# Fil/nd4js

Measured on AMD Instinct MI355X. Metric: fp64 GFLOP/s: matmul N=4096 & SVD N=2048; % of MFMA/HBM peak, higher is better.
Workload: dtype f64; 1 GPU; matmul 4096x4096x4096 fp64, one matrix pair per GPU (BASELINE configs[1]); parallelism=batch-sharded x1, no collective, inputs=uniform(-1,1) seeds 5/6, HBM-resident

## Files before the change

nd4js_amd/csrc/gemm.hip:

```cpp
#include "nd4hip_internal.h"
#include <cstdlib>

typedef double d4 __attribute__((ext_vector_type(4)));
typedef double d2 __attribute__((ext_vector_type(2)));

namespace {

constexpr int BM = 128, BN = 128, BK = 16;
constexpr int LDR = BK + 1;
constexpr int LDK = BN + 16;
constexpr int TILE = BK * LDK;
constexpr int NXCD = 8, GROUP_M = 8;

struct GemmArgs {
  const double* A; const double* B; double* C;
  int M, N, K;
  long lda, ldb, ldc, sA, sB, sC;
  double alpha, beta;
  int tiles_m, tiles_n;
  int lower;
  int kchunk;
  double* Cpart;
};

template <bool VEC, bool FULL>
__device__ __forceinline__ void load_row(d2 (&r)[4], const double* __restrict__ P, long ld,
                                         int x0, int X, int k0, int K, int t) {
  const int kc = k0 + ((t & 7) << 1);
#pragma unroll
  for (int q = 0; q < 4; q++) {
    const int x = x0 + q * 32 + (t >> 3);
    const double* p = P + (long)x * ld + kc;
    if (FULL) {
      r[q] = *reinterpret_cast<const d2*>(p);
    } else if (VEC) {
      d2 v = {0.0, 0.0};
      if (x < X && kc < K) v = *reinterpret_cast<const d2*>(p);
      r[q] = v;
    } else {
      double a = 0.0, b = 0.0;
      if (x < X && kc < K) a = p[0];
      if (x < X && kc + 1 < K) b = p[1];
      r[q].x = a; r[q].y = b;
    }
  }
}
__device__ __forceinline__ void store_row(double* S, const d2 (&r)[4], int t) {
  const int kc = (t & 7) << 1;
#pragma unroll
  for (int q = 0; q < 4; q++) {
    double* s = S + (q * 32 + (t >> 3)) * LDR + kc;
    s[0] = r[q].x; s[1] = r[q].y;
  }
}
template <bool VEC, bool FULL>
__device__ __forceinline__ void load_kmaj(d2 (&r)[4], const double* __restrict__ P, long ld,
                                          int x0, int X, int k0, int K, int t) {
  const int k = k0 + (t >> 4);
#pragma unroll
  for (int q = 0; q < 4; q++) {
    const int x = x0 + q * 32 + ((t & 15) << 1);
    const double* p = P + (long)k * ld + x;
    if (FULL) {
      r[q] = *reinterpret_cast<const d2*>(p);
    } else if (VEC) {
      d2 v = {0.0, 0.0};
      if (k < K && x < X) v = *reinterpret_cast<const d2*>(p);
      r[q] = v;
    } else {
      double a = 0.0, b = 0.0;
      if (k < K && x < X) a = p[0];
      if (k < K && x + 1 < X) b = p[1];
      r[q].x = a; r[q].y = b;
    }
  }
}
__device__ __forceinline__ void store_kmaj(double* S, const d2 (&r)[4], int t) {
#pragma unroll
  for (int q = 0; q < 4; q++)
    *reinterpret_cast<d2*>(S + (t >> 4) * LDK + q * 32 + ((t & 15) << 1)) = r[q];
}

template <bool FULL, bool BETA>
__device__ __forceinline__ void store_c(const d4 (&acc)[4][4], double* __restrict__ c0, long ldc, int rows, int cols, double alpha, double beta) {
#pragma unroll
  for (int i = 0; i < 4; i++)
#pragma unroll
    for (int j = 0; j < 4; j++)
#pragma unroll
      for (int r = 0; r < 4; r++)
        if (FULL || (i * 16 + 4 * r < rows && j * 16 < cols)) {
          double* c = c0 + (long)(i * 16 + 4 * r) * ldc + j * 16;
          double v = alpha * acc[i][j][r];
          if (BETA) v += beta * *c;
          *c = v;
        }
}

template <bool TA, bool TB, bool VEC, bool FULL>
__global__ __launch_bounds__(256, 2) void dgemm_kernel(GemmArgs g) {
  __shared__ __attribute__((aligned(16))) double lds[4 * TILE];

  const int nwg = g.tiles_m * g.tiles_n;
  int wg;
  {
    const int bid = blockIdx.x, xcd = bid % NXCD, within = bid / NXCD;
    const int q = nwg / NXCD, r = nwg % NXCD;
    wg = (xcd < r ? xcd * (q + 1) : r * (q + 1) + (xcd - r) * q) + within;
  }
  const int per_group = GROUP_M * g.tiles_n;
  const int first_m = (wg / per_group) * GROUP_M;
  const int gsz = min(g.tiles_m - first_m, GROUP_M);
  const int tm = first_m + (wg % per_group) % gsz;
  const int tn = (wg % per_group) / gsz;
  const int m0 = tm * BM, n0 = tn * BN;
  if (g.lower && n0 > m0 + BM - 1) return;

  const long bz = blockIdx.y;
  const double* __restrict__ A = g.A + bz * g.sA;
  const double* __restrict__ B = g.B + bz * g.sB;
  double* __restrict__ C = g.C + bz * g.sC;
  int kbeg = 0, kend = g.K;
  long ldc = g.ldc;
  double alpha = g.alpha, beta = g.beta;
  if (g.kchunk > 0) {
    kbeg = blockIdx.z * g.kchunk; kend = min(g.K, kbeg + g.kchunk);
    C = g.Cpart + ((long)blockIdx.z * gridDim.y + bz) * g.M * g.N;
    ldc = g.N; alpha = 1.0; beta = 0.0;
  }

  const int t = threadIdx.x, lane = t & 63, wave = t >> 6;
  const int wm = (wave >> 1) * 64, wn = (wave & 1) * 64;
  const int fx = lane & 15, fk = lane >> 4;

  d4 acc[4][4];
#pragma unroll
  for (int i = 0; i < 4; i++)
#pragma unroll
    for (int j = 0; j < 4; j++) acc[i][j] = d4{0.0, 0.0, 0.0, 0.0};

  d2 ra[4], rb[4];
  auto gload = [&](int k0) {
    if (TA) load_kmaj<VEC, FULL>(ra, A, g.lda, m0, g.M, k0, kend, t); else load_row<VEC, FULL>(ra, A, g.lda, m0, g.M, k0, kend, t);
    if (TB) load_row<VEC, FULL>(rb, B, g.ldb, n0, g.N, k0, kend, t);  else load_kmaj<VEC, FULL>(rb, B, g.ldb, n0, g.N, k0, kend, t);
  };
  auto sstore = [&](int buf) {
    double* sa = lds + buf * 2 * TILE; double* sb = sa + TILE;
    if (TA) store_kmaj(sa, ra, t); else store_row(sa, ra, t);
    if (TB) store_row(sb, rb, t);  else store_kmaj(sb, rb, t);
  };

  const double* fa = lds + (TA ? fk * LDK + wm + fx : (wm + fx) * LDR + fk);
  const double* fb = lds + TILE + (TB ? (wn + fx) * LDR + fk : fk * LDK + wn + fx);
  auto fread = [&](double (&a)[4], double (&b)[4], int buf, int kk) __attribute__((always_inline)) {
#pragma unroll
    for (int i = 0; i < 4; i++) a[i] = fa[buf * 2 * TILE + (TA ? kk * 4 * LDK + i * 16 : i * 16 * LDR + kk * 4)];
#pragma unroll
    for (int j = 0; j < 4; j++) b[j] = fb[buf * 2 * TILE + (TB ? j * 16 * LDR + kk * 4 : kk * 4 * LDK + j * 16)];
    __builtin_amdgcn_sched_barrier(0);
  };
  auto mma = [&](const double (&a)[4], const double (&b)[4]) __attribute__((always_inline)) {
#pragma unroll
    for (int i = 0; i < 4; i++)
#pragma unroll
      for (int j = 0; j < 4; j++)
        acc[i][j] = __builtin_amdgcn_mfma_f64_16x16x4f64(a[i], b[j], acc[i][j], 0, 0, 0);
    __builtin_amdgcn_sched_barrier(0);
  };

  const int nk = (kend - kbeg + BK - 1) / BK;
  gload(kbeg);
  sstore(0);
  if (nk > 1) gload(kbeg + BK);
  __syncthreads();

  double a0[4], b0[4], a1[4], b1[4];
  fread(a0, b0, 0, 0);
  auto kstep = [&](int cur, int kt, bool more, bool more2) __attribute__((always_inline)) {
    fread(a1, b1, cur, 1); mma(a0, b0);
    fread(a0, b0, cur, 2); mma(a1, b1);
    fread(a1, b1, cur, 3);
    if (more) { sstore(cur ^ 1); __builtin_amdgcn_sched_barrier(0); }
    mma(a0, b0);
    if (more) {
      __syncthreads();
      if (more2) gload(kbeg + (kt + 2) * BK);
      fread(a0, b0, cur ^ 1, 0);
    }
    mma(a1, b1);
  };
  int kt = 0;
  for (; kt + 2 < nk; kt += 2) {
    kstep(0, kt, true, true);
    kstep(1, kt + 1, true, kt + 3 < nk);
  }
  if (kt < nk) kstep(0, kt, kt + 1 < nk, false);
  if (kt + 1 < nk) kstep(1, kt + 1, false, false);

  double* c0 = C + (long)(m0 + wm + fk) * ldc + n0 + wn + fx;
  if (beta != 0.0) store_c<FULL, true>(acc, c0, ldc, g.M - (m0 + wm + fk), g.N - (n0 + wn + fx), alpha, beta);
  else             store_c<FULL, false>(acc, c0, ldc, g.M - (m0 + wm + fk), g.N - (n0 + wn + fx), alpha, beta);
}

constexpr int SK_RT = 1;
constexpr int SK_CT = 2;
constexpr int SK_BM = 4 * 16 * SK_RT, SK_BN = 16 * SK_CT, SK_KSTEPS = 8;

template <bool TB>
__global__ __launch_bounds__(256, 4) void dgemm_smallk_kernel(GemmArgs g) {
  const int tm = blockIdx.x / g.tiles_n, tn = blockIdx.x % g.tiles_n;
  const int m0 = tm * SK_BM, n0 = tn * SK_BN;
  if (g.lower && n0 > m0 + SK_BM - 1) return;
  const int lane = threadIdx.x & 63, w = threadIdx.x >> 6;
  const int fx = lane & 15, fk = lane >> 4;
  const int rbase = m0 + w * 16 * SK_RT;
  if (rbase >= g.M) return;
  const long bz = blockIdx.y;
  const double* __restrict__ A = g.A + bz * g.sA;
  const double* __restrict__ B = g.B + bz * g.sB;
  double* __restrict__ C = g.C + bz * g.sC;
  const int nk = (g.K + 3) >> 2;

  d4 acc[SK_RT][SK_CT];
  const double scale = (g.beta == 0.0) ? 0.0 : g.beta / g.alpha;
#pragma unroll
  for (int i = 0; i < SK_RT; i++)
#pragma unroll
    for (int j = 0; j < SK_CT; j++) {
      const int col = n0 + j * 16 + fx;
#pragma unroll
      for (int r = 0; r < 4; r++) {
        const int row = rbase + i * 16 + fk + 4 * r;
        double c = 0.0;
        if (scale != 0.0 && row < g.M && col < g.N) c = scale * C[(long)row * g.ldc + col];
        acc[i][j][r] = c;
      }
    }
  double a[SK_RT][SK_KSTEPS], b[SK_CT][SK_KSTEPS];
#pragma unroll
  for (int i = 0; i < SK_RT; i++) {
    const int row = rbase + i * 16 + fx;
    const double* ap = A + (long)row * g.lda + fk;
#pragma unroll
    for (int kk = 0; kk < SK_KSTEPS; kk++) a[i][kk] = (row < g.M && kk * 4 + fk < g.K) ? ap[kk * 4] : 0.0;
  }
#pragma unroll
  for (int j = 0; j < SK_CT; j++) {
    const int col = n0 + j * 16 + fx;
#pragma unroll
    for (int kk = 0; kk < SK_KSTEPS; kk++) {
      const int k = kk * 4 + fk;
      double v = 0.0;
      if (col < g.N && k < g.K) v = TB ? B[(long)col * g.ldb + k] : B[(long)k * g.ldb + col];
      b[j][kk] = v;
    }
  }
#pragma unroll
  for (int kk = 0; kk < SK_KSTEPS; kk++)
    if (kk < nk) {
#pragma unroll
      for (int i = 0; i < SK_RT; i++)
#pragma unroll
        for (int j = 0; j < SK_CT; j++) acc[i][j] = __builtin_amdgcn_mfma_f64_16x16x4f64(a[i][kk], b[j][kk], acc[i][j], 0, 0, 0);
    }
  const double alpha = g.alpha;
#pragma unroll
  for (int i = 0; i < SK_RT; i++)
#pragma unroll
    for (int j = 0; j < SK_CT; j++) {
      const int col = n0 + j * 16 + fx;
#pragma unroll
      for (int r = 0; r < 4; r++) {
        const int row = rbase + i * 16 + fk + 4 * r;
        if (row < g.M && col < g.N) C[(long)row * g.ldc + col] = alpha * acc[i][j][r];
      }
    }
}

bool smallk_ok(const GemmArgs& g, bool transA) {
  return !transA && g.K >= 1 && g.K <= 4 * SK_KSTEPS && (g.alpha == 1.0 || g.alpha == -1.0) &&
         (g.beta == 0.0 || g.beta == 1.0 || g.beta == -1.0);
}
template <bool TB>
int launch_smallk(nd4hip_handle* h, GemmArgs g, int64_t batch) {
  g.tiles_m = (g.M + SK_BM - 1) / SK_BM; g.tiles_n = (g.N + SK_BN - 1) / SK_BN;
  ND4_CHECK_ARG((int64_t)g.tiles_m * g.tiles_n < (1ll << 31), "nd4_gemm: too many tiles");
  hipLaunchKernelGGL((dgemm_smallk_kernel<TB>), dim3((unsigned)(g.tiles_m * g.tiles_n), (unsigned)batch, 1), dim3(256, 1, 1), 0, h->stream, g);
  ND4_HIP(hipGetLastError());
  return 0;
}

__global__ __launch_bounds__(256) void dgemm_splitk_reduce(const double* __restrict__ part, int nsplit, long per_split, int M, int N,
                                                            double alpha, double beta, double* __restrict__ Cm, long ldc, long sC) {
  const long b = blockIdx.y;
  const long e = blockIdx.x * 256l + threadIdx.x;
  if (e >= (long)M * N) return;
  double s = 0.0;
  for (int z = 0; z < nsplit; z++) s += part[z * per_split + b * (long)M * N + e];
  double* c = Cm + b * sC + (e / N) * ldc + e % N;
  double v = alpha * s;
  if (beta != 0.0) v += beta * *c;
  *c = v;
}


template <bool TA, bool TB>
int launch(nd4hip_handle* h, const GemmArgs& g, bool vec, int64_t batch) {
  const unsigned nsplit = g.kchunk > 0 ? (unsigned)((g.K + g.kchunk - 1) / g.kchunk) : 1u;
  dim3 grid((unsigned)(g.tiles_m * g.tiles_n), (unsigned)batch, nsplit), block(256, 1, 1);
  const bool full = vec && g.M % BM == 0 && g.N % BN == 0 && g.K % BK == 0 && g.K > 0;
  if (full)     hipLaunchKernelGGL((dgemm_kernel<TA, TB, true, true>), grid, block, 0, h->stream, g);
  else if (vec) hipLaunchKernelGGL((dgemm_kernel<TA, TB, true, false>), grid, block, 0, h->stream, g);
  else          hipLaunchKernelGGL((dgemm_kernel<TA, TB, false, false>), grid, block, 0, h->stream, g);
  ND4_HIP(hipGetLastError());
  return 0;
}

}

int nd4_gemm(nd4hip_handle* h, bool transA, bool transB, int64_t M, int64_t N, int64_t K,
             double alpha, const double* A, int64_t lda, int64_t sA,
             const double* B, int64_t ldb, int64_t sB,
             double beta, double* C, int64_t ldc, int64_t sC, int64_t batch) {
  if (M <= 0 || N <= 0 || batch <= 0) return 0;
  ND4_CHECK_ARG(K >= 0 && M < (1 << 30) && N < (1 << 30) && K < (1 << 30), "nd4_gemm: extent out of range");
  ND4_CHECK_ARG(batch <= 65535, "nd4_gemm: batch %lld exceeds 65535 per launch", (long long)batch);
  GemmArgs g;
  g.A = A; g.B = B; g.C = C; g.M = (int)M; g.N = (int)N; g.K = (int)K;
  g.lda = lda; g.ldb = ldb; g.ldc = ldc; g.sA = sA; g.sB = sB; g.sC = sC;
  g.alpha = alpha; g.beta = beta; g.lower = 0; g.kchunk = 0; g.Cpart = nullptr;
  g.tiles_m = (int)((M + BM - 1) / BM); g.tiles_n = (int)((N + BN - 1) / BN);
  ND4_CHECK_ARG((int64_t)g.tiles_m * g.tiles_n < (1ll << 31), "nd4_gemm: too many tiles");
  if (smallk_ok(g, transA)) return transB ? launch_smallk<true>(h, g, batch) : launch_smallk<false>(h, g, batch);
  Nd4WsScope scope(h);
  const int64_t tiles = (int64_t)g.tiles_m * g.tiles_n * batch;
  int nsplit = 1;
  if (tiles <= 160 && K >= 512) {
    int64_t want = 384 / tiles;
    if (want > K / 256) want = K / 256;
    if (want > 32) want = 32;
    if (want >= 2) {
      int64_t kc = ((K + want - 1) / want + BK - 1) / BK * BK;
      nsplit = (int)((K + kc - 1) / kc);
      void* p = nullptr;
      ND4_TRY(nd4_ws_alloc(h, sizeof(double) * (size_t)nsplit * (size_t)batch * (size_t)M * (size_t)N, &p));
      g.kchunk = (int)kc; g.Cpart = static_cast<double*>(p);
    }
  }
  auto even = [](int64_t v) { return (v & 1) == 0; };
  auto al16 = [](const void* p) { return (reinterpret_cast<uintptr_t>(p) & 15) == 0; };
  const bool vec = al16(A) && al16(B) && even(lda) && even(ldb) && even(sA) && even(sB) &&
                   even(transA ? M : K) && even(transB ? K : N);
  if (transA) ND4_TRY((transB ? launch<true, true>(h, g, vec, batch) : launch<true, false>(h, g, vec, batch)));
  else        ND4_TRY((transB ? launch<false, true>(h, g, vec, batch) : launch<false, false>(h, g, vec, batch)));
  if (g.kchunk > 0) {
    hipLaunchKernelGGL(dgemm_splitk_reduce, dim3((unsigned)((M * N + 255) / 256), (unsigned)batch), dim3(256), 0, h->stream,
                       g.Cpart, nsplit, (long)batch * M * N, (int)M, (int)N, alpha, beta, C, (long)ldc, (long)sC);
    ND4_HIP(hipGetLastError());
  }
  return 0;
}

int nd4_syrk_lower(nd4hip_handle* h, int64_t N, int64_t K, double alpha, const double* A, int64_t lda, int64_t sA,
                   double beta, double* C, int64_t ldc, int64_t sC, int64_t batch) {
  return nd4_gemm_nt_lower(h, N, K, alpha, A, lda, sA, A, lda, sA, beta, C, ldc, sC, batch);
}
int nd4_gemm_nt_lower(nd4hip_handle* h, int64_t N, int64_t K, double alpha, const double* A, int64_t lda, int64_t sA,
                      const double* B, int64_t ldb, int64_t sB, double beta, double* C, int64_t ldc, int64_t sC, int64_t batch) {
  if (N <= 0 || batch <= 0) return 0;
  ND4_CHECK_ARG(K >= 0 && N < (1 << 30) && K < (1 << 30), "nd4_gemm_nt_lower: extent out of range");
  ND4_CHECK_ARG(batch <= 65535, "nd4_gemm_nt_lower: batch %lld exceeds 65535 per launch", (long long)batch);
  GemmArgs g;
  g.A = A; g.B = B; g.C = C; g.M = (int)N; g.N = (int)N; g.K = (int)K;
  g.lda = lda; g.ldb = ldb; g.ldc = ldc; g.sA = sA; g.sB = sB; g.sC = sC;
  g.alpha = alpha; g.beta = beta; g.lower = 1; g.kchunk = 0; g.Cpart = nullptr;
  if (smallk_ok(g, false)) return launch_smallk<true>(h, g, batch);
  g.tiles_m = (int)((N + BM - 1) / BM); g.tiles_n = g.tiles_m;
  auto ok = [](const double* p, int64_t ld, int64_t st) { return (reinterpret_cast<uintptr_t>(p) & 15) == 0 && (ld & 1) == 0 && (st & 1) == 0; };
  const bool vec = ok(A, lda, sA) && ok(B, ldb, sB) && (K & 1) == 0;
  return launch<false, true>(h, g, vec, batch);
}
```

Baseline: 70950 GFLOP/s.

## Make DGEMM kernel persistent with grid-stride tile walk and prefetched next tile

Replaces the one-workgroup-per-tile launch with a persistent grid sized to resident occupancy times CU count. Each workgroup walks tiles, batches and split-K chunks with a grid stride, and loads the next tile's first K slice before storing the current C tile. The aim is to cut workgroup launch and tail overhead and to overlap the epilogue with the next tile's loads. It adds per-item index math read from the kernarg segment and optional timestamp instrumentation behind a compile flag. It may also disturb the XCD/group-M tile mapping locality for 4096 matrices.

New measurement: 67840 GFLOP/s. 4.4% lower.

```diff
diff --git a/nd4js_amd/csrc/gemm.hip b/nd4js_amd/csrc/gemm.hip
--- a/nd4js_amd/csrc/gemm.hip
+++ b/nd4js_amd/csrc/gemm.hip
@@ -21,7 +21,20 @@
   int lower;
   int kchunk;
   double* Cpart;
+  int batch, work;
+#ifdef ND4_GEMM_STAMPS
+  unsigned long long* stamps;
+#endif
 };
+
+#ifdef ND4_GEMM_STAMPS
+constexpr int STAMP_WORDS = 32;
+unsigned long long* g_stamps = nullptr;
+int g_stamps_one_trip = 0;
+#define ND4_STAMP(i) do { if (st && t == 0) { __builtin_amdgcn_sched_barrier(0); st[i] = wall_clock64(); __builtin_amdgcn_sched_barrier(0); } } while (0)
+#else
+#define ND4_STAMP(i) do { } while (0)
+#endif
 
 template <bool VEC, bool FULL>
 __device__ __forceinline__ void load_row(d2 (&r)[4], const double* __restrict__ P, long ld,
@@ -101,44 +114,47 @@
 __global__ __launch_bounds__(256, 2) void dgemm_kernel(GemmArgs g) {
   __shared__ __attribute__((aligned(16))) double lds[4 * TILE];
 
-  const int nwg = g.tiles_m * g.tiles_n;
-  int wg;
-  {
-    const int bid = blockIdx.x, xcd = bid % NXCD, within = bid / NXCD;
+  int m0, n0, kbeg, kend;
+  const double* A; const double* B; double* C;
+  const long ldc = g.kchunk > 0 ? g.N : g.ldc;
+  const double alpha = g.kchunk > 0 ? 1.0 : g.alpha, beta = g.kchunk > 0 ? 0.0 : g.beta;
+  typedef const __attribute__((address_space(4))) GemmArgs* KernArgs;
+  auto item = [&](int v) {
+    KernArgs ka = (KernArgs)__builtin_amdgcn_kernarg_segment_ptr();
+    asm volatile("" : "+s"(ka));
+    const int tiles_m = ka->tiles_m, tiles_n = ka->tiles_n, nwg = tiles_m * tiles_n, batch = ka->batch, kchunk = ka->kchunk;
+    const int bid = v % nwg, rest = v / nwg, xcd = bid % NXCD, within = bid / NXCD;
     const int q = nwg / NXCD, r = nwg % NXCD;
-    wg = (xcd < r ? xcd * (q + 1) : r * (q + 1) + (xcd - r) * q) + within;
-  }
-  const int per_group = GROUP_M * g.tiles_n;
-  const int first_m = (wg / per_group) * GROUP_M;
-  const int gsz = min(g.tiles_m - first_m, GROUP_M);
-  const int tm = first_m + (wg % per_group) % gsz;
-  const int tn = (wg % per_group) / gsz;
-  const int m0 = tm * BM, n0 = tn * BN;
-  if (g.lower && n0 > m0 + BM - 1) return;
-
-  const long bz = blockIdx.y;
-  const double* __restrict__ A = g.A + bz * g.sA;
-  const double* __restrict__ B = g.B + bz * g.sB;
-  double* __restrict__ C = g.C + bz * g.sC;
-  int kbeg = 0, kend = g.K;
-  long ldc = g.ldc;
-  double alpha = g.alpha, beta = g.beta;
-  if (g.kchunk > 0) {
-    kbeg = blockIdx.z * g.kchunk; kend = min(g.K, kbeg + g.kchunk);
-    C = g.Cpart + ((long)blockIdx.z * gridDim.y + bz) * g.M * g.N;
-    ldc = g.N; alpha = 1.0; beta = 0.0;
-  }
+    const int wg = (xcd < r ? xcd * (q + 1) : r * (q + 1) + (xcd - r) * q) + within;
+    const int per_group = GROUP_M * tiles_n;
+    const int first_m = (wg / per_group) * GROUP_M;
+    const int gsz = min(tiles_m - first_m, GROUP_M);
+    m0 = (first_m + (wg % per_group) % gsz) * BM;
+    n0 = ((wg % per_group) / gsz) * BN;
+    const long bz = rest % batch, z = rest / batch;
+    A = ka->A + bz * ka->sA; B = ka->B + bz * ka->sB; C = ka->C + bz * ka->sC;
+    kbeg = 0; kend = ka->K;
+    if (kchunk > 0) {
+      kbeg = (int)z * kchunk; kend = min(kend, kbeg + kchunk);
+      C = ka->Cpart + (z * batch + bz) * ka->M * ka->N;
+    }
+    return !(ka->lower && n0 > m0 + BM - 1);
+  };
+  auto next_item = [&](int v) {
+    KernArgs ka = (KernArgs)__builtin_amdgcn_kernarg_segment_ptr();
+    asm volatile("" : "+s"(ka));
+    for (const int work = ka->work; v < work; v += gridDim.x)
+      if (item(v)) return v;
+    return -1;
+  };
+  int v = next_item(blockIdx.x);
+  if (v < 0) return;
 
   const int t = threadIdx.x, lane = t & 63, wave = t >> 6;
   const int wm = (wave >> 1) * 64, wn = (wave & 1) * 64;
   const int fx = lane & 15, fk = lane >> 4;
 
   d4 acc[4][4];
-#pragma unroll
-  for (int i = 0; i < 4; i++)
-#pragma unroll
-    for (int j = 0; j < 4; j++) acc[i][j] = d4{0.0, 0.0, 0.0, 0.0};
-
   d2 ra[4], rb[4];
   auto gload = [&](int k0) {
     if (TA) load_kmaj<VEC, FULL>(ra, A, g.lda, m0, g.M, k0, kend, t); else load_row<VEC, FULL>(ra, A, g.lda, m0, g.M, k0, kend, t);
@@ -168,14 +184,16 @@
     __builtin_amdgcn_sched_barrier(0);
   };
 
-  const int nk = (kend - kbeg + BK - 1) / BK;
+#ifdef ND4_GEMM_STAMPS
+  unsigned long long* st = g.stamps ? g.stamps + (size_t)blockIdx.x * STAMP_WORDS : nullptr;
+  int nitem = 0;
+  ND4_STAMP(0);
+  if (st && t == 0) st[1] = (unsigned long long)__builtin_amdgcn_s_getreg((31 << 11) | 4) | (unsigned long long)__builtin_amdgcn_s_getreg((31 << 11) | 20) << 32;
+#endif
+  int nk;
   gload(kbeg);
   sstore(0);
-  if (nk > 1) gload(kbeg + BK);
-  __syncthreads();
-
   double a0[4], b0[4], a1[4], b1[4];
-  fread(a0, b0, 0, 0);
   auto kstep = [&](int cur, int kt, bool more, bool more2) __attribute__((always_inline)) {
     fread(a1, b1, cur, 1); mma(a0, b0);
     fread(a0, b0, cur, 2); mma(a1, b1);
@@ -189,17 +207,47 @@
     }
     mma(a1, b1);
   };
-  int kt = 0;
-  for (; kt + 2 < nk; kt += 2) {
-    kstep(0, kt, true, true);
-    kstep(1, kt + 1, true, kt + 3 < nk);
-  }
-  if (kt < nk) kstep(0, kt, kt + 1 < nk, false);
-  if (kt + 1 < nk) kstep(1, kt + 1, false, false);
-
-  double* c0 = C + (long)(m0 + wm + fk) * ldc + n0 + wn + fx;
-  if (beta != 0.0) store_c<FULL, true>(acc, c0, ldc, g.M - (m0 + wm + fk), g.N - (n0 + wn + fx), alpha, beta);
-  else             store_c<FULL, false>(acc, c0, ldc, g.M - (m0 + wm + fk), g.N - (n0 + wn + fx), alpha, beta);
+  for (;;) {
+    nk = (kend - kbeg + BK - 1) / BK;
+    if (nk > 1) gload(kbeg + BK);
+    __syncthreads();
+#pragma unroll
+    for (int i = 0; i < 4; i++)
+#pragma unroll
+      for (int j = 0; j < 4; j++) acc[i][j] = d4{0.0, 0.0, 0.0, 0.0};
+    fread(a0, b0, 0, 0);
+#ifdef ND4_GEMM_STAMPS
+    if (nitem < 9) ND4_STAMP(4 + 3 * nitem);
+#endif
+
+    int kt = 0;
+    for (; kt + 2 < nk; kt += 2) {
+      kstep(0, kt, true, true);
+      kstep(1, kt + 1, true, kt + 3 < nk);
+    }
+    if (kt < nk) kstep(0, kt, kt + 1 < nk, false);
+    if (kt + 1 < nk) kstep(1, kt + 1, false, false);
+#ifdef ND4_GEMM_STAMPS
+    if (nitem < 9) ND4_STAMP(5 + 3 * nitem);
+#endif
+
+    double* c0 = C + (long)(m0 + wm + fk) * ldc + n0 + wn + fx;
+    const int rows = g.M - (m0 + wm + fk), cols = g.N - (n0 + wn + fx);
+    v = next_item(v + gridDim.x);
+    if (v >= 0) gload(kbeg);
+    if (beta != 0.0) store_c<FULL, true>(acc, c0, ldc, rows, cols, alpha, beta);
+    else             store_c<FULL, false>(acc, c0, ldc, rows, cols, alpha, beta);
+#ifdef ND4_GEMM_STAMPS
+    if (nitem < 9) ND4_STAMP(6 + 3 * nitem);
+    nitem++;
+#endif
+    if (v < 0) break;
+    __syncthreads();
+    sstore(0);
+  }
+#ifdef ND4_GEMM_STAMPS
+  if (st && t == 0) { __builtin_amdgcn_s_waitcnt(0); st[3] = wall_clock64(); st[2] = (unsigned long long)nitem; }
+#endif
 }
 
 constexpr int SK_RT = 1;
@@ -304,16 +352,42 @@
 }
 
 
-template <bool TA, bool TB>
-int launch(nd4hip_handle* h, const GemmArgs& g, bool vec, int64_t batch) {
-  const unsigned nsplit = g.kchunk > 0 ? (unsigned)((g.K + g.kchunk - 1) / g.kchunk) : 1u;
-  dim3 grid((unsigned)(g.tiles_m * g.tiles_n), (unsigned)batch, nsplit), block(256, 1, 1);
-  const bool full = vec && g.M % BM == 0 && g.N % BN == 0 && g.K % BK == 0 && g.K > 0;
-  if (full)     hipLaunchKernelGGL((dgemm_kernel<TA, TB, true, true>), grid, block, 0, h->stream, g);
-  else if (vec) hipLaunchKernelGGL((dgemm_kernel<TA, TB, true, false>), grid, block, 0, h->stream, g);
-  else          hipLaunchKernelGGL((dgemm_kernel<TA, TB, false, false>), grid, block, 0, h->stream, g);
+template <bool TA, bool TB, bool VEC, bool FULL>
+int resident_per_cu(int* out) {
+  static int occ = 0;
+  if (occ == 0) {
+    int n = 0;
+    ND4_HIP(hipOccupancyMaxActiveBlocksPerMultiprocessor(&n, dgemm_kernel<TA, TB, VEC, FULL>, 256, 0));
+    occ = n < 1 ? 1 : n;
+  }
+  *out = occ;
+  return 0;
+}
+template <bool TA, bool TB, bool VEC, bool FULL>
+int launch_walk(nd4hip_handle* h, GemmArgs g) {
+  int occ = 0;
+  ND4_TRY((resident_per_cu<TA, TB, VEC, FULL>(&occ)));
+  long grid = (long)occ * h->num_cu;
+  if (g.work <= grid) grid = g.work;
+  else if (grid > NXCD) grid -= grid % NXCD;
+#ifdef ND4_GEMM_STAMPS
+  g.stamps = g_stamps;
+  if (g_stamps_one_trip) grid = g.work;
+#endif
+  hipLaunchKernelGGL((dgemm_kernel<TA, TB, VEC, FULL>), dim3((unsigned)grid, 1, 1), dim3(256, 1, 1), 0, h->stream, g);
   ND4_HIP(hipGetLastError());
   return 0;
+}
+template <bool TA, bool TB>
+int launch(nd4hip_handle* h, GemmArgs g, bool vec, int64_t batch) {
+  const int64_t nsplit = g.kchunk > 0 ? (g.K + g.kchunk - 1) / g.kchunk : 1;
+  const int64_t work = (int64_t)g.tiles_m * g.tiles_n * batch * nsplit;
+  ND4_CHECK_ARG(work < (1ll << 30), "nd4_gemm: too many tiles");
+  g.batch = (int)batch; g.work = (int)work;
+  const bool full = vec && g.M % BM == 0 && g.N % BN == 0 && g.K % BK == 0 && g.K > 0;
+  if (full) return launch_walk<TA, TB, true, true>(h, g);
+  if (vec)  return launch_walk<TA, TB, true, false>(h, g);
+  return launch_walk<TA, TB, false, false>(h, g);
 }
 
 }
@@ -380,3 +454,7 @@
   const bool vec = ok(A, lda, sA) && ok(B, ldb, sB) && (K & 1) == 0;
   return launch<false, true>(h, g, vec, batch);
 }
+
+#ifdef ND4_GEMM_STAMPS
+extern "C" void nd4_gemm_stamps(unsigned long long* buf, int one_trip) { g_stamps = buf; g_stamps_one_trip = one_trip; }
+#endif
```

## Add persistent dgemm variant that prefetches the next tile during the C epilogue

Applied to the files above, without the earlier changes.

Adds a resident-grid (persistent) variant of the fp64 MFMA GEMM kernel, launched with 2×CU workgroups rounded to a multiple of the XCD count. Each workgroup walks over tiles and batch entries with a fixed stride. Before writing back the current tile's C, it issues the global loads and LDS store for the next tile, so the epilogue overlaps with the next prologue and the tail between launch waves is avoided. It is only used for full, non-split-K, non-lower shapes that have more tiles than resident slots. The cost is extra loop-carried state and a changed tile-to-CU assignment that could shift L2 locality.

Result: slower. 70760 GFLOP/s before, 69970 GFLOP/s after (-1.1%).

```diff
diff --git a/nd4js_amd/csrc/gemm.hip b/nd4js_amd/csrc/gemm.hip
--- a/nd4js_amd/csrc/gemm.hip
+++ b/nd4js_amd/csrc/gemm.hip
@@ -21,7 +21,20 @@
   int lower;
   int kchunk;
   double* Cpart;
+  int batch;
+  int step_q, step_r;
 };
+
+__device__ __forceinline__ void tile_origin(const GemmArgs& g, int nwg, int bid, int& m0, int& n0) {
+  const int xcd = bid % NXCD, within = bid / NXCD;
+  const int q = nwg / NXCD, r = nwg % NXCD;
+  const int wg = (xcd < r ? xcd * (q + 1) : r * (q + 1) + (xcd - r) * q) + within;
+  const int per_group = GROUP_M * g.tiles_n;
+  const int first_m = (wg / per_group) * GROUP_M;
+  const int gsz = min(g.tiles_m - first_m, GROUP_M);
+  m0 = (first_m + (wg % per_group) % gsz) * BM;
+  n0 = ((wg % per_group) / gsz) * BN;
+}
 
 template <bool VEC, bool FULL>
 __device__ __forceinline__ void load_row(d2 (&r)[4], const double* __restrict__ P, long ld,
@@ -97,26 +110,17 @@
         }
 }
 
-template <bool TA, bool TB, bool VEC, bool FULL>
+template <bool TA, bool TB, bool VEC, bool FULL, bool RES>
 __global__ __launch_bounds__(256, 2) void dgemm_kernel(GemmArgs g) {
   __shared__ __attribute__((aligned(16))) double lds[4 * TILE];
 
   const int nwg = g.tiles_m * g.tiles_n;
-  int wg;
-  {
-    const int bid = blockIdx.x, xcd = bid % NXCD, within = bid / NXCD;
-    const int q = nwg / NXCD, r = nwg % NXCD;
-    wg = (xcd < r ? xcd * (q + 1) : r * (q + 1) + (xcd - r) * q) + within;
-  }
-  const int per_group = GROUP_M * g.tiles_n;
-  const int first_m = (wg / per_group) * GROUP_M;
-  const int gsz = min(g.tiles_m - first_m, GROUP_M);
-  const int tm = first_m + (wg % per_group) % gsz;
-  const int tn = (wg % per_group) / gsz;
-  const int m0 = tm * BM, n0 = tn * BN;
+  int bid = RES ? (int)(blockIdx.x % (unsigned)nwg) : (int)blockIdx.x;
+  int m0, n0;
+  tile_origin(g, nwg, bid, m0, n0);
   if (g.lower && n0 > m0 + BM - 1) return;
 
-  const long bz = blockIdx.y;
+  long bz = RES ? (long)(blockIdx.x / (unsigned)nwg) : (long)blockIdx.y;
   const double* __restrict__ A = g.A + bz * g.sA;
   const double* __restrict__ B = g.B + bz * g.sB;
   double* __restrict__ C = g.C + bz * g.sC;
@@ -169,6 +173,7 @@
   };
 
   const int nk = (kend - kbeg + BK - 1) / BK;
+  if (RES) asm volatile("" :: "s"(g.batch), "s"(g.step_q), "s"(g.step_r));
   gload(kbeg);
   sstore(0);
   if (nk > 1) gload(kbeg + BK);
@@ -189,17 +194,42 @@
     }
     mma(a1, b1);
   };
-  int kt = 0;
-  for (; kt + 2 < nk; kt += 2) {
-    kstep(0, kt, true, true);
-    kstep(1, kt + 1, true, kt + 3 < nk);
-  }
-  if (kt < nk) kstep(0, kt, kt + 1 < nk, false);
-  if (kt + 1 < nk) kstep(1, kt + 1, false, false);
-
-  double* c0 = C + (long)(m0 + wm + fk) * ldc + n0 + wn + fx;
-  if (beta != 0.0) store_c<FULL, true>(acc, c0, ldc, g.M - (m0 + wm + fk), g.N - (n0 + wn + fx), alpha, beta);
-  else             store_c<FULL, false>(acc, c0, ldc, g.M - (m0 + wm + fk), g.N - (n0 + wn + fx), alpha, beta);
+  for (;;) {
+    int kt = 0;
+    for (; kt + 2 < nk; kt += 2) {
+      kstep(0, kt, true, true);
+      kstep(1, kt + 1, true, kt + 3 < nk);
+    }
+    if (kt < nk) kstep(0, kt, kt + 1 < nk, false);
+    if (kt + 1 < nk) kstep(1, kt + 1, false, false);
+
+    double* c0 = C + (long)(m0 + wm + fk) * ldc + n0 + wn + fx;
+    const int crows = g.M - (m0 + wm + fk), ccols = g.N - (n0 + wn + fx);
+    bool next = false;
+    if (RES) {
+      bid += g.step_r; bz += g.step_q;
+      if (bid >= nwg) { bid -= nwg; bz++; }
+      next = bz < g.batch;
+      if (next) {
+        tile_origin(g, nwg, bid, m0, n0);
+        A = g.A + bz * g.sA; B = g.B + bz * g.sB; C = g.C + bz * g.sC;
+        gload(kbeg);
+        if (nk & 1) __syncthreads();
+        sstore(0);
+        if (nk > 1) gload(kbeg + BK);
+        __builtin_amdgcn_sched_barrier(0);
+      }
+    }
+    if (beta != 0.0) store_c<FULL, true>(acc, c0, ldc, crows, ccols, alpha, beta);
+    else             store_c<FULL, false>(acc, c0, ldc, crows, ccols, alpha, beta);
+    if (!RES || !next) break;
+#pragma unroll
+    for (int i = 0; i < 4; i++)
+#pragma unroll
+      for (int j = 0; j < 4; j++) acc[i][j] = d4{0.0, 0.0, 0.0, 0.0};
+    __syncthreads();
+    fread(a0, b0, 0, 0);
+  }
 }
 
 constexpr int SK_RT = 1;
@@ -305,13 +335,18 @@
 
 
 template <bool TA, bool TB>
-int launch(nd4hip_handle* h, const GemmArgs& g, bool vec, int64_t batch) {
+int launch(nd4hip_handle* h, GemmArgs g, bool vec, int64_t batch) {
   const unsigned nsplit = g.kchunk > 0 ? (unsigned)((g.K + g.kchunk - 1) / g.kchunk) : 1u;
   dim3 grid((unsigned)(g.tiles_m * g.tiles_n), (unsigned)batch, nsplit), block(256, 1, 1);
   const bool full = vec && g.M % BM == 0 && g.N % BN == 0 && g.K % BK == 0 && g.K > 0;
-  if (full)     hipLaunchKernelGGL((dgemm_kernel<TA, TB, true, true>), grid, block, 0, h->stream, g);
-  else if (vec) hipLaunchKernelGGL((dgemm_kernel<TA, TB, true, false>), grid, block, 0, h->stream, g);
-  else          hipLaunchKernelGGL((dgemm_kernel<TA, TB, false, false>), grid, block, 0, h->stream, g);
+  const unsigned resident = (unsigned)(2 * h->num_cu / NXCD * NXCD);
+  const int64_t nwg = (int64_t)g.tiles_m * g.tiles_n;
+  g.batch = (int)batch; g.step_q = (int)(resident / nwg); g.step_r = (int)(resident % nwg);
+  if (full && g.kchunk == 0 && !g.lower && resident > 0 && nwg * batch > (int64_t)resident)
+                hipLaunchKernelGGL((dgemm_kernel<TA, TB, true, true, true>), dim3(resident, 1, 1), block, 0, h->stream, g);
+  else if (full) hipLaunchKernelGGL((dgemm_kernel<TA, TB, true, true, false>), grid, block, 0, h->stream, g);
+  else if (vec)  hipLaunchKernelGGL((dgemm_kernel<TA, TB, true, false, false>), grid, block, 0, h->stream, g);
+  else           hipLaunchKernelGGL((dgemm_kernel<TA, TB, false, false, false>), grid, block, 0, h->stream, g);
   ND4_HIP(hipGetLastError());
   return 0;
 }
@@ -328,7 +363,7 @@
   GemmArgs g;
   g.A = A; g.B = B; g.C = C; g.M = (int)M; g.N = (int)N; g.K = (int)K;
   g.lda = lda; g.ldb = ldb; g.ldc = ldc; g.sA = sA; g.sB = sB; g.sC = sC;
-  g.alpha = alpha; g.beta = beta; g.lower = 0; g.kchunk = 0; g.Cpart = nullptr;
+  g.alpha = alpha; g.beta = beta; g.lower = 0; g.kchunk = 0; g.Cpart = nullptr; g.batch = (int)batch; g.step_q = g.step_r = 0;
   g.tiles_m = (int)((M + BM - 1) / BM); g.tiles_n = (int)((N + BN - 1) / BN);
   ND4_CHECK_ARG((int64_t)g.tiles_m * g.tiles_n < (1ll << 31), "nd4_gemm: too many tiles");
   if (smallk_ok(g, transA)) return transB ? launch_smallk<true>(h, g, batch) : launch_smallk<false>(h, g, batch);
@@ -373,7 +408,7 @@
   GemmArgs g;
   g.A = A; g.B = B; g.C = C; g.M = (int)N; g.N = (int)N; g.K = (int)K;
   g.lda = lda; g.ldb = ldb; g.ldc = ldc; g.sA = sA; g.sB = sB; g.sC = sC;
-  g.alpha = alpha; g.beta = beta; g.lower = 1; g.kchunk = 0; g.Cpart = nullptr;
+  g.alpha = alpha; g.beta = beta; g.lower = 1; g.kchunk = 0; g.Cpart = nullptr; g.batch = (int)batch; g.step_q = g.step_r = 0;
   if (smallk_ok(g, false)) return launch_smallk<true>(h, g, batch);
   g.tiles_m = (int)((N + BM - 1) / BM); g.tiles_n = g.tiles_m;
   auto ok = [](const double* p, int64_t ld, int64_t st) { return (reinterpret_cast<uintptr_t>(p) & 15) == 0 && (ld & 1) == 0 && (st & 1) == 0; };
```
